# MiroBeno/Volume-Rendering

Hardware: AMD Instinct MI355X
Metric: Mrays/s (W*H / t_frame), 1024^3 volume @ 2048^2 viewport (higher is better)
Workload: dtype f32

## Files before the change

### __graft_entry__.py

```python
import importlib
import os
import subprocess
import sys

ROOT = os.path.dirname(os.path.abspath(__file__))
PKG = "volume-rendering_amd"


def load_package():
    if ROOT not in sys.path:
        sys.path.insert(0, ROOT)
    return importlib.import_module(PKG)


def build():
    subprocess.check_call(["make", "-C", os.path.join(ROOT, PKG, "csrc")])
    os.makedirs(os.path.join(ROOT, "build_variants"), exist_ok=True)
    subprocess.check_call(["bash", os.path.join(ROOT, "scripts", "build_variant.sh"), "bounds", "-DVR_BOUNDS_CHECK"], stdout=subprocess.DEVNULL)
    subprocess.check_call(["make", "-C", os.path.join(ROOT, "oracle"), "oracle"])
    if os.path.isdir("/root/reference/VolumeRendering"):
        subprocess.check_call(["make", "-C", os.path.join(ROOT, "oracle"), "ref"])
        subprocess.check_call(["make", "-C", os.path.join(ROOT, "oracle"), "binding"])
    vr = load_package()
    vr.lib()


def smoke():
    import numpy as np
    import torch

    assert torch.cuda.is_available(), "smoke() needs an MI355X"
    sys.path.insert(0, os.path.join(ROOT, "tests"))
    from helpers import Golden, Oracle, compare_frames
# ... 28 lines not shown
```

### volume-rendering_amd/csrc/vr_device.h

```cpp
#pragma once

#include <hip/hip_runtime.h>
#include <stdint.h>
#include "../../include/vr_hip.h"

namespace vr {

constexpr uint32_t kMaxRaySteps = 1u << 22;

#ifndef VR_DEPTH
#define VR_DEPTH 5
#endif
constexpr int kDepth = VR_DEPTH, kSlots = kDepth + 1;
#ifndef VR_LAZY_EXIT
#define VR_LAZY_EXIT 1
#endif
#ifndef VR_RUN_DEPTH
#define VR_RUN_DEPTH VR_DEPTH
#endif
constexpr int kDepthTwoByte = 3;
constexpr int kRunDepth = VR_RUN_DEPTH, kMaxDepth = kRunDepth > kDepth ? kRunDepth : kDepth;
constexpr int kOverrunSteps = kMaxDepth + (VR_LAZY_EXIT ? kMaxDepth + 1 : 0);
constexpr int kLutPad = (kOverrunSteps * 5 + 2) / 3 + 2;
static_assert(kDepth >= 1 && kDepth <= 6 && kRunDepth >= 1 && kRunDepth <= 12, "prefetch depth");
// ... 140 lines not shown
hipError_t launch_brickify_voxel(const void *linear, void *voxel_bricks, uint32_t bytes_per_voxel, uint32_t dim_x, uint32_t dim_y, uint32_t dim_z,
                                 hipStream_t stream);
hipError_t launch_brickify_oct(const void *linear, void *oct_bricks, uint32_t dim_x, uint32_t dim_y, uint32_t dim_z, hipStream_t stream);
hipError_t launch_brickify_run(const void *linear, void *run_copy, uint32_t run_layout , uint32_t dim_x, uint32_t dim_y,
                               uint32_t dim_z, hipStream_t stream);
hipError_t launch_build_column(const void *linear, void *col_copy, uint32_t axis, bool voxels , uint32_t dim_x, uint32_t dim_y, uint32_t dim_z, hipStream_t stream);
inline uint64_t bricked_elems(uint32_t dim_x, uint32_t dim_y, uint32_t dim_z) {
	return (uint64_t) ((dim_x + kBrickEdge - 1) / kBrickEdge) * ((dim_y + kBrickEdge - 1) / kBrickEdge) *
	       ((dim_z + kBrickEdge - 1) / kBrickEdge) * kBrickPitch;
}

hipError_t launch_raymarch(const RayKernelArgs &a, const void *linear, const void *bricked, uint32_t bytes_per_voxel,
                           const float *tf_premult , const uint32_t *esl_bits ,
                           void *out_rgba, TileSchedule sched, hipStream_t stream);
hipError_t launch_colmarch(const RayKernelArgs &a, const void *copy, const float *tf_premult, void *out_rgba, hipStream_t stream);

struct RaymarchPlan { bool reads_linear; uint32_t tiles_x, tiles_y; uint32_t tile_h = 16;  };
RaymarchPlan plan_raymarch(const RayKernelArgs &a, bool have_bricked, uint32_t bytes_per_voxel);
hipError_t launch_tile_order(uint32_t *cost, uint32_t *order, uint32_t ntiles, hipStream_t stream);
hipError_t launch_tile_estimate(const RayKernelArgs &a, uint32_t tile_h, const uint32_t *esl, uint32_t *cost, uint32_t ntiles, hipStream_t stream);
hipError_t launch_tile_choice(const uint32_t *cost_z, const uint32_t *cost_y, uint32_t *choice, uint32_t ntiles, hipStream_t stream);

hipError_t launch_minmax(const void *volume, uint32_t bytes_per_voxel, uint32_t dim_x, uint32_t dim_y, uint32_t dim_z,
                         uint32_t esl_block_dims, uint8_t *minmax_dev , hipStream_t stream);

constexpr uint32_t kMipBoundEntries = VR_ESL_VOLUME_DIMS * VR_ESL_VOLUME_DIMS * VR_ESL_VOLUME_DIMS;
constexpr uint32_t kMipStatsAt = 2u * kMipBoundEntries + 16u, kMipBoundBytes = kMipStatsAt + 16u;
hipError_t launch_mip_bounds(const uint8_t *minmax_dev , uint8_t *bounds_dev , hipStream_t stream);
hipError_t launch_mip(const RayKernelArgs &a, const void *linear, const void *bricked, uint32_t bytes_per_voxel, const float *tf_premult,
                      const uint8_t *bounds, void *out_rgba, hipStream_t stream);
// ... 12 lines not shown
```

### volume-rendering_amd/csrc/vr_hip_api.cpp

```cpp
#include "vr_device.h"

#include <algorithm>
#include <chrono>
#include <cmath>
#include <cstdio>
#include <cstdlib>
#include <cstring>
#include <new>
#include <string>
#include <vector>

using namespace vr;

#ifndef VR_ORDER_ALWAYS
#define VR_ORDER_ALWAYS 0
#endif

namespace {

constexpr int kEventRing = 256;

struct EventPair { hipEvent_t start = nullptr, stop = nullptr; bool pending = false; };

}
// ... 1249 lines not shown
}

#ifdef VR_MIP_STATS
int vr_hip_debug_mip_stats(vr_ctx *c, uint64_t *out2) {
	if (c == nullptr || out2 == nullptr) return VR_ERR_INVALID;
	out2[0] = out2[1] = 0;
	if (!c->mip_bounds_ready) return VR_OK;
	VR_TRY(c, hipSetDevice(c->device));
	VR_TRY(c, drain(c));
	VR_TRY(c, hipMemcpy(out2, c->mip_bounds + kMipStatsAt, 16, hipMemcpyDeviceToHost));
	VR_TRY(c, hipMemset(c->mip_bounds + kMipStatsAt, 0, 16));
	return VR_OK;
}
#endif

int vr_hip_timing(vr_ctx *c, vr_timing *out) {
	if (c == nullptr || out == nullptr) return VR_ERR_INVALID;
	(void) hipSetDevice(c->device);
	for (int i = 0; i < kEventRing; i++)
		harvest(c, c->ring[(c->ring_head + i) % kEventRing]);
	out->kernel_ms = c->last_kernel_ms;
	out->total_ms = c->last_total_ms > 0 ? c->last_total_ms : c->last_kernel_ms;
	out->launches = c->launches;
	out->kernel_ms_sum = c->kernel_ms_sum;
	out->kernel_ms_max = c->kernel_ms_max;
	out->total_ms_max = c->total_ms_max;
	return VR_OK;
}

int vr_hip_timing_reset(vr_ctx *c) {
// ... 157 lines not shown
```

### volume-rendering_amd/csrc/vr_kernels.hip

```cpp
#include "vr_march.h"

namespace vr {

#ifndef VR_COL_DEPTH
#define VR_COL_DEPTH 3
#endif
#ifndef VR_COL_WAVES
#define VR_COL_WAVES 4
#endif
constexpr int kColDepth = VR_COL_DEPTH, kColSlots = kColDepth + 1;

__device__ __forceinline__ void managed_load128_s(u32x4 &dst, uint32_t byte_offset, uint64_t base) {
	asm volatile("global_load_dwordx4 %0, %1, %2" : "=&v"(dst) : "v"(byte_offset), "s"(base));
}
template <int I> __device__ __forceinline__ float comp3(const f3 &v) { return I == 0 ? v.x : (I == 1 ? v.y : v.z); }

template <int M, bool Q8>
__device__ __forceinline__ float col_resolve(uint32_t w0, uint32_t w1, float max_x, float max_y, float max_z, float xb, float yb, float zb) {
	const float ax = filter_weight<Q8>(__builtin_amdgcn_fractf(__builtin_amdgcn_fmed3f(xb, 0.0f, max_x)));
	const float ay = filter_weight<Q8>(__builtin_amdgcn_fractf(__builtin_amdgcn_fmed3f(yb, 0.0f, max_y)));
	const float az = filter_weight<Q8>(__builtin_amdgcn_fractf(__builtin_amdgcn_fmed3f(zb, 0.0f, max_z)));
	const float p0 = (float) (w0 & 0xffu), p1 = (float) ((w0 >> 8) & 0xffu), p2 = (float) ((w0 >> 16) & 0xffu), p3 = (float) (w0 >> 24);
	const float q0 = (float) (w1 & 0xffu), q1 = (float) ((w1 >> 8) & 0xffu), q2 = (float) ((w1 >> 16) & 0xffu), q3 = (float) (w1 >> 24);
	float v000, v100, v010, v110, v001, v101, v011, v111;
// ... 1 lines not shown
	else if (M == 1) { v000 = p0; v100 = p1; v001 = p2; v101 = p3; v010 = q0; v110 = q1; v011 = q2; v111 = q3; }
	else             { v000 = p0; v010 = p1; v001 = p2; v011 = p3; v100 = q0; v110 = q1; v101 = q2; v111 = q3; }
	const float c00 = lerp(v000, v100, ax), c10 = lerp(v010, v110, ax);
	const float c01 = lerp(v001, v101, ax), c11 = lerp(v011, v111, ax);
	const float c0 = lerp(c00, c10, ay), c1 = lerp(c01, c11, ay);
	return lerp(c0, c1, az);
}


typedef const RayKernelArgs __attribute__((address_space(4))) *ColConstArgs;
struct ColKernelArguments { RayKernelArgs a; const uint8_t *copy; const float *tf_g; uint32_t *out; };
typedef const ColKernelArguments __attribute__((address_space(4))) *ColConstKernelArguments;
__device__ __forceinline__ ColConstArgs col_dense_args() { ColConstArgs q = (ColConstArgs) __builtin_amdgcn_kernarg_segment_ptr(); asm volatile("" : "+s"(q)); return q; }
__device__ __forceinline__ float uni(float v) { return __uint_as_float(rfl(__float_as_uint(v))); }
__device__ __forceinline__ uint32_t col_lane_id() { return __builtin_amdgcn_mbcnt_hi(~0u, __builtin_amdgcn_mbcnt_lo(~0u, 0u)); }

__device__ __forceinline__ void stage_tf_with_deltas(f4 (&tf_l)[VR_TF_SIZE + 1], f4 (&dtf_l)[VR_TF_SIZE + 1], const float *__restrict__ tf_g) {
	const uint32_t t = threadIdx.x;
	if (t <= VR_TF_SIZE) {
		const f4 *tf4 = (const f4 *) tf_g;
		const uint32_t i0 = t < VR_TF_SIZE ? t : VR_TF_SIZE - 1, i1 = t + 1 < VR_TF_SIZE ? t + 1 : VR_TF_SIZE - 1;
		const f4 c0 = tf4[i0], c1 = tf4[i1];
		tf_l[t] = c0;
		f4 d; d.x = c1.x - c0.x; d.y = c1.y - c0.y; d.z = c1.z - c0.z; d.w = c1.w - c0.w;
		dtf_l[t] = d;
	}
}

struct ColRay {
	bool in_frame, alive;
	uint32_t out_index;
	uint32_t org_slot;
	f3 dir, origin;
	float kx, ky, step;
	uint64_t alive_mask;
};
__device__ __forceinline__ f3 col_origin_again(const f4 (&org_l)[512], uint32_t &org_slot) {
	pin(org_slot);
	const f4 o4 = *(const f4 *) ((const char *) org_l + org_slot);
	return mk3(o4.x, o4.y, o4.z);
}
__device__ __forceinline__ void col_ray_setup(const RayKernelArgs &a, f4 (&org_l)[512], ColRay &r) {
	uint32_t tile_x, tile_y;
	tile_to_xy<VR_COL_XCD_MODE>(a.tiles_x, a.tiles_y, blockIdx.x, blockIdx.x, tile_x, tile_y);
	uint32_t lx, ly;
	lane_pixel<512u, true>(a, tile_x, tile_y, lx, ly);
	r.in_frame = lx < a.p.out_width && ly < a.p.out_rows;
	r.out_index = r.in_frame ? ly * a.p.out_width + lx : 0xffffffffu;

	const PixelRay ray = pixel_ray<true>(a, a.p.x0 + lx, frame_row(a, ly));
	r.dir = ray.dir; r.origin = ray.origin;
	r.org_slot = threadIdx.x * (uint32_t) sizeof(f4);
	{ f4 o4; o4.x = r.origin.x; o4.y = r.origin.y; o4.z = r.origin.z; o4.w = 0.0f; org_l[threadIdx.x] = o4; }
	r.kx = ray.kx; r.ky = ray.ky;
	r.step = a.p.ray_step;
	const bool alive = r.in_frame && ray.alive;
	r.alive = alive;
	r.alive_mask = __builtin_amdgcn_ballot_w64(alive);
	if (!alive) r.ky = -1.0f;
}

struct ColWave {
	int leader;
	float kx_l, cm_l;
	int cu0, cv0, cu1, cv1;
	uint64_t flips_u, flips_v;
	bool ok;
};
template <class CellU, class CellV>
__device__ __forceinline__ void col_wave_eligibility(const ColRay &r, float cm, float advance, CellU cell_u, CellV cell_v, ColWave &w) {
	w.leader = __builtin_ctzll(r.alive_mask);
	w.kx_l = rlane(r.kx, w.leader); w.cm_l = rlane(cm, w.leader);
	w.ok = __builtin_amdgcn_ballot_w64(r.alive && (__float_as_uint(r.kx) != __float_as_uint(w.kx_l) || __float_as_uint(cm) != __float_as_uint(w.cm_l))) == 0ull;
	w.ok = w.ok && __builtin_amdgcn_ballot_w64(!(advance >= (1.0f / 64.0f) && advance <= 1.0f)) == 0ull;
	w.cu0 = cell_u(r.kx); w.cv0 = cell_v(r.kx);
	w.cu1 = cell_u(r.ky); w.cv1 = cell_v(r.ky);
	{
		const int lu = __builtin_amdgcn_readlane(w.cu0, w.leader), lv = __builtin_amdgcn_readlane(w.cv0, w.leader);
		if (!r.alive) { w.cu0 = w.cu1 = lu; w.cv0 = w.cv1 = lv; }
	}
	w.flips_u = __builtin_amdgcn_ballot_w64(w.cu0 != w.cu1); w.flips_v = __builtin_amdgcn_ballot_w64(w.cv0 != w.cv1);
	w.ok = w.ok && __builtin_amdgcn_ballot_w64((w.cu1 - w.cu0) * (w.cu1 - w.cu0) > 1 || (w.cv1 - w.cv0) * (w.cv1 - w.cv0) > 1) == 0ull;
}
__device__ __forceinline__ bool col_lane_offsets(const ColWave &w, uint64_t stride_u, uint64_t stride_v, int64_t &ref, int64_t &rel0) {
	ref = (int64_t) col_lateral_offset64((uint32_t) __builtin_amdgcn_readlane(w.cu0, w.leader), (uint32_t) __builtin_amdgcn_readlane(w.cv0, w.leader), stride_u, stride_v);
	rel0 = (int64_t) col_lateral_offset64((uint32_t) w.cu0, (uint32_t) w.cv0, stride_u, stride_v) - ref;
	const int64_t du64 = (int64_t) col_axis_offset64((uint32_t) w.cu1, stride_u, kColWindowBytes) - (int64_t) col_axis_offset64((uint32_t) w.cu0, stride_u, kColWindowBytes);
	const int64_t dv64 = (int64_t) col_axis_offset64((uint32_t) w.cv1, stride_v, kColRowBytes) - (int64_t) col_axis_offset64((uint32_t) w.cv0, stride_v, kColRowBytes);
	const int64_t lim = 1ll << 28;
	return __builtin_amdgcn_ballot_w64(rel0 <= -lim || rel0 >= lim || du64 <= -lim || du64 >= lim || dv64 <= -lim || dv64 >= lim) == 0ull;
}
__device__ __forceinline__ uint64_t col_scalar_base(const uint8_t *copy, int64_t ref) {
	const uint64_t b = (uint64_t) (uintptr_t) copy + (uint64_t) ref - (1ull << 30);
	return ((uint64_t) rfl((uint32_t) (b >> 32)) << 32) | rfl((uint32_t) b);
// ... 198 lines not shown
__device__ __forceinline__ void col_drain(u32x4 (&slot)[N], More &...more) {
	static_for<0, N>([&](auto j) { pin(slot[j.value]); });
	if constexpr (sizeof...(More) != 0) pin(more...);
	managed_wait<0>();
	static_for<0, N>([&](auto j) { pin(slot[j.value]); });
	if constexpr (sizeof...(More) != 0) pin(more...);
}
__device__ __forceinline__ void col_store(const ColRay &ray, const f4 &acc) {
	uint32_t ky_bits = __float_as_uint(ray.ky), out_index = ray.out_index;
	pin(ky_bits, out_index);
	uint32_t rgba = 0;
	if (__uint_as_float(ky_bits) > 0.0f) rgba = map_float_int(acc.x, 256) | (map_float_int(acc.y, 256) << 8) | (map_float_int(acc.z, 256) << 16) | (map_float_int(acc.w, 256) << 24);
	if (out_index != 0xffffffffu) ((ColConstKernelArguments) col_dense_args())->out[out_index] = rgba;
}

template <int SAMPLING, int M, bool FLIPS>
__global__ __launch_bounds__(512) __attribute__((amdgpu_waves_per_eu(VR_COL_WAVES, 8)))
void colmarch_kernel(const RayKernelArgs a, const uint8_t *__restrict__ copy, const float *__restrict__ tf_g, uint32_t *__restrict__ out) {
	constexpr int U = M == 0 ? 1 : 0, V = M == 2 ? 1 : 2;
	__shared__ f4 tf_l[VR_TF_SIZE + 1], dtf_l[VR_TF_SIZE + 1];
	__shared__ f4 org_l[512];
	stage_tf_with_deltas(tf_l, dtf_l, tf_g);
	__syncthreads();
	ColRay ray;
	col_ray_setup(a, org_l, ray);
	if (ray.alive_mask == 0ull) { if (ray.in_frame) out[ray.out_index] = 0u; return; }

	const f3 A = mk3(uni(ray.dir.x * a.half_x), uni(ray.dir.y * a.half_y), uni(ray.dir.z * a.half_z));
	const f3 B = mk3(VR_FMA(ray.origin.x, a.half_x, a.off_x), VR_FMA(ray.origin.y, a.half_y, a.off_y), VR_FMA(ray.origin.z, a.half_z, a.off_z));
	const float Am = comp3<M>(A), Au = comp3<U>(A), Av = comp3<V>(A);
	const float Bm = comp3<M>(B), Bu = comp3<U>(B), Bv = comp3<V>(B);
	const uint32_t dim_u = U == 0 ? a.dim_x : a.dim_y, dim_m = M == 0 ? a.dim_x : (M == 1 ? a.dim_y : a.dim_z);
	const float max_u = U == 0 ? a.max_x : a.max_y, max_v = V == 1 ? a.max_y : a.max_z;
	const uint32_t nbu = col_blocks(dim_u), nw = col_windows(dim_m);
	const uint64_t stride_u = (uint64_t) nw * kColBlockBytes, stride_v = (uint64_t) nbu * stride_u;

	f4 acc; acc.x = acc.y = acc.z = acc.w = 0.0f;
	uint64_t live = ray.alive_mask;
	float k = ray.kx;

	auto coords = [&](ColConstArgs q, float kk, float &xb, float &yb, float &zb) {
// ... 12 lines not shown
		coords(q, kk, xb, yb, zb);
		managed_load64(both, (uint64_t) (uintptr_t) col_pair_address<M>(a, ((ColConstKernelArguments) q)->copy, q->col_sample.max_x, q->col_sample.max_y, q->col_sample.max_z, q->col_shade.nbu, q->col_shade.nw, xb, yb, zb));
	};
	auto sample = [&](uint32_t w0, uint32_t w1) {
		col_tri_sample<SAMPLING, M>(a, w0, w1, k, B, ray, live, acc, tf_l, dtf_l, org_l,
			[&](const uint8_t *copy_p, const RayKernelArgs::ColDenseSample &ds, const RayKernelArgs::ColDenseShade &dh, float sx, float sy, float sz, uint32_t &l0, uint32_t &l1) {
				const uint2 both = *(const uint2 *) col_pair_address<M>(a, copy_p, ds.max_x, ds.max_y, ds.max_z, dh.nbu, dh.nw, sx, sy, sz);
				l0 = both.x; l1 = both.y;
			});
	};

	auto cell = [&](float kk, float Ac, float Bc, float maxc) { return (int) __builtin_amdgcn_fmed3f(VR_FMA(kk, Ac, Bc), 0.0f, maxc); };
	auto cell_u = [&](float kk) { return cell(kk, Au, Bu, max_u); };
	auto cell_v = [&](float kk) { return cell(kk, Av, Bv, max_v); };
	ColWave wv;
	col_wave_eligibility(ray, Bm, __builtin_fabsf(Am) * ray.step, cell_u, cell_v, wv);
	int64_t ref, rel0;
	const bool ok = col_lane_offsets(wv, stride_u, stride_v, ref, rel0) && wv.ok;
	const float Bm_l = wv.cm_l;

	const bool has_flips = (wv.flips_u | wv.flips_v) != 0ull;
	auto per_lane_march = [&]() {
		while (live != 0ull) {
			uint32_t w0, w1;
			fetch_at(k, w0, w1);
			sample(w0, w1);
			k += ray.step;
			live &= __builtin_amdgcn_fcmpf(k, ray.ky, kFcmpOLE);
		}
	};
	if (ok) {
		const uint32_t voff0 = (uint32_t) (rel0 + (1ll << 30));
		const uint64_t s_base = col_scalar_base(copy, ref);
		const int dsign = (__float_as_uint(comp3<M>(ray.dir)) >> 31) != 0u ? -1 : 1;
		auto window_of = [](int lc) { return (int) (__umulhi((uint32_t) lc + 0x30000000u, 0xAAAAAAABu) >> 1) - 0x10000000; };
		auto cell_window = [&](float kk) { return window_of((int) VR_FMA(kk, Am, Bm_l)); };
		int key_u = kColNoEvent, key_v = kColNoEvent;
// ... 39 lines not shown
						} else {
							const uint32_t sub = rfl((uint32_t) (int) VR_FMA(k, Am, Bm_l)) - first;
							sample(sub == 0u ? o.x : (sub == 1u ? o.y : o.z), sub == 0u ? o.y : (sub == 1u ? o.z : o.w));
						}
					});
				}
				cur += dsign;
			};
			while (live != 0ull && guard > 0) {
				static_for<0, kColSlots>(window_step);
				guard -= kColSlots;
			}
			col_drain(slot);
		}
	} else per_lane_march();
	col_store(ray, acc);
}

__device__ __forceinline__ void managed_load8_at(uint32_t &dst, uint64_t address) {
	asm volatile("global_load_ubyte %0, %1, off" : "=&v"(dst) : "v"(address));
}

template <int M, bool FLIPS>
__global__ __launch_bounds__(512) __attribute__((amdgpu_waves_per_eu(VR_COL_WAVES, 8)))
void colmarch_nearest_kernel(const RayKernelArgs a, const uint8_t *__restrict__ copy, const float *__restrict__ tf_g, uint32_t *__restrict__ out) {
	constexpr int U = M == 0 ? 1 : 0, V = M == 2 ? 1 : 2;
	constexpr int kCells = (int) kColVoxCells;
	__shared__ f4 tf_l[VR_TF_SIZE];
	__shared__ float unit_l[256];
	__shared__ f4 org_l[512];
	{
		const uint32_t t = threadIdx.x;
		if (t < VR_TF_SIZE) tf_l[t] = ((const f4 *) tf_g)[t];
		if (t < 256u) unit_l[t] = (float) t / 255.0f;
	}
	__syncthreads();
	ColRay ray;
	col_ray_setup(a, org_l, ray);
	if (ray.alive_mask == 0ull) { if (ray.in_frame) out[ray.out_index] = 0u; return; }

	const float dm = comp3<M>(ray.dir), du = comp3<U>(ray.dir), dv = comp3<V>(ray.dir);
	const float om = comp3<M>(ray.origin), ou = comp3<U>(ray.origin), ov = comp3<V>(ray.origin);
	const uint32_t dim_u = U == 0 ? a.dim_x : a.dim_y, dim_v = V == 1 ? a.dim_y : a.dim_z, dim_m = M == 0 ? a.dim_x : (M == 1 ? a.dim_y : a.dim_z);
	const float half_m = M == 0 ? a.half_x : (M == 1 ? a.half_y : a.half_z);
	const uint32_t nbu = col_blocks(dim_u), nw = col_windows(dim_m, kColVoxCells);
	const uint64_t stride_u = (uint64_t) nw * kColBlockBytes, stride_v = (uint64_t) nbu * stride_u;

	f4 acc; acc.x = acc.y = acc.z = acc.w = 0.0f;
	uint64_t live = ray.alive_mask;
	float k = ray.kx;
	const int opaque_above = ((int) a.tf_zero_below + 1) * VR_TF_RATIO - 1;
	uint32_t near_mask = 0u, near_cmp = 1u;
	if (opaque_above >= 0) { const uint32_t p2 = 1u << (31 - __builtin_clz((uint32_t) opaque_above + 1u)); near_mask = (0xffu & ~(p2 - 1u)) * 0x01010101u; near_cmp = 0u; }

// ... 39 lines not shown
				const float sl = unit_l[s_l], sc = unit_l[s & 255u];
				const float diffuse = select_lanes(shaded, (sl - sc) * kd);
				cur.x += diffuse; cur.y += diffuse; cur.z += diffuse;
			}
			const float t = select_lanes(live, 1 - acc.w);
			acc.x = acc.x + cur.x * t; acc.y = acc.y + cur.y * t;
			acc.z = acc.z + cur.z * t; acc.w = acc.w + cur.w * t;
			live &= ~__builtin_amdgcn_fcmpf(acc.w, threshold, kFcmpOGT);
		}
	};

	auto cell_lat = [&](float kk, float oc, float dc, uint32_t n) { return (int) map_float_int(((oc + dc * kk) + 1) * 0.5f, n); };
	auto cell_u = [&](float kk) { return cell_lat(kk, ou, du, dim_u); };
	auto cell_v = [&](float kk) { return cell_lat(kk, ov, dv, dim_v); };
	ColWave wv;
	col_wave_eligibility(ray, om, __builtin_fabsf(dm * half_m) * ray.step, cell_u, cell_v, wv);
	int64_t ref, rel0;
	const bool ok = col_lane_offsets(wv, stride_u, stride_v, ref, rel0) && wv.ok;
	const float om_l = wv.cm_l;
	auto cell_m = [&](float kk) { const int c = (int) (((om_l + dm * kk) + 1.0f) * half_m); return c == (int) dim_m ? (int) dim_m - 1 : c; };
	const bool has_flips = (wv.flips_u | wv.flips_v) != 0ull;
	auto per_lane_march = [&]() {
		while (live != 0ull) {
			ColConstArgs q = col_dense_args();
			const uint32_t s = *voxel_address_at(q, position(q, k));
			sample(s);
			k += ray.step;
			live &= __builtin_amdgcn_fcmpf(k, ray.ky, kFcmpOLE);
		}
	};
	if (ok) {
		const uint32_t voff0 = (uint32_t) (rel0 + (1ll << 30));
		const uint64_t s_base = col_scalar_base(copy, ref);
		const int dsign = (__float_as_uint(dm) >> 31) != 0u ? -1 : 1;
		auto cell_window = [&](float kk) { return cell_m(kk) >> 4; };
		int key_u = kColNoEvent, key_v = kColNoEvent;
		if (FLIPS && wv.flips_u != 0ull) key_u = wv.cu0 != wv.cu1 ? dsign * cell_window(__uint_as_float(col_bisect(ray, wv.cu0 != wv.cu1, wv.cu0, cell_u))) : kColNoEvent;
// ... 40 lines not shown
							const uint32_t sub = (uint32_t) ((int) rfl((uint32_t) cell_m(k)) - first) & 15u;
							const uint32_t word = (sub >> 2) == 0u ? o.x : ((sub >> 2) == 1u ? o.y : ((sub >> 2) == 2u ? o.z : o.w));
							sample((word >> ((sub & 3u) * 8u)) & 0xffu);
						}
					});
				}
				cur += dsign;
			};
			while (live != 0ull && guard > 0) {
				static_for<0, kColSlots>(window_step);
				guard -= kColSlots;
			}
			col_drain(slot);
		}
	} else per_lane_march();
	col_store(ray, acc);
}

#ifndef VR_VOXCOL_DEPTH
#define VR_VOXCOL_DEPTH 3
#endif
#ifndef VR_VOXCOL_WAVES
#define VR_VOXCOL_WAVES VR_COL_WAVES
#endif
constexpr int kVoxColDepth = VR_VOXCOL_DEPTH, kVoxColSlots = kVoxColDepth + 1;
static_assert(kVoxColDepth >= 2 && 2 * kVoxColSlots + kVoxColDepth + 4 <= 64, "kColPadBytes");

template <int SAMPLING, int M, bool FLIPS, bool PAIRS>
__device__ __forceinline__ void voxcol_march(const RayKernelArgs &a, const uint8_t *__restrict__ copy, const float *__restrict__ tf_g, uint32_t *__restrict__ out,
                                             f4 (&tf_l)[VR_TF_SIZE + 1], f4 (&dtf_l)[VR_TF_SIZE + 1], f4 (&org_l)[512]) {
	constexpr int U = M == 0 ? 1 : 0, V = M == 2 ? 1 : 2;
	constexpr int kCells = (int) kColVoxCells;
	stage_tf_with_deltas(tf_l, dtf_l, tf_g);
	__syncthreads();
	ColRay ray;
	col_ray_setup(a, org_l, ray);
	if (ray.alive_mask == 0ull) { if (ray.in_frame) out[ray.out_index] = 0u; return; }

	const f3 A = mk3(uni(ray.dir.x * a.half_x), uni(ray.dir.y * a.half_y), uni(ray.dir.z * a.half_z));
	const f3 B = mk3(VR_FMA(ray.origin.x, a.half_x, a.off_x), VR_FMA(ray.origin.y, a.half_y, a.off_y), VR_FMA(ray.origin.z, a.half_z, a.off_z));
	const float Am = comp3<M>(A), Au = comp3<U>(A), Av = comp3<V>(A);
	const float Bm = comp3<M>(B), Bu = comp3<U>(B), Bv = comp3<V>(B);
	const uint32_t dim_u = U == 0 ? a.dim_x : a.dim_y, dim_v = V == 1 ? a.dim_y : a.dim_z, dim_m = M == 0 ? a.dim_x : (M == 1 ? a.dim_y : a.dim_z);
	const float max_u = U == 0 ? a.max_x : a.max_y, max_v = V == 1 ? a.max_y : a.max_z;
	const uint32_t nbu = col_blocks(dim_u), nw = col_windows(dim_m, kColVoxCells);
	const uint64_t stride_u = (uint64_t) nw * kColBlockBytes, stride_v = (uint64_t) nbu * stride_u;

	f4 acc; acc.x = acc.y = acc.z = acc.w = 0.0f;
	uint64_t live = ray.alive_mask;
	float k = ray.kx;

	auto corners_at = [&](const uint8_t *copy_p, float mx, float my, float mz, uint32_t blocks_u, uint32_t windows, float xb, float yb, float zb,
	                      uint32_t &w0, uint32_t &w1) {
		if constexpr (PAIRS) {
			const uint2 both = *(const uint2 *) col_pair_address<M>(a, copy_p, mx, my, mz, blocks_u, windows, xb, yb, zb);
			w0 = both.x; w1 = both.y;
			return;
		}
		const uint32_t ix = (uint32_t) (int) __builtin_amdgcn_fmed3f(xb, 0.0f, mx), iy = (uint32_t) (int) __builtin_amdgcn_fmed3f(yb, 0.0f, my),
		               iz = (uint32_t) (int) __builtin_amdgcn_fmed3f(zb, 0.0f, mz);
		const float fu = U == 0 ? mx : my, fv = V == 1 ? my : mz, fm = M == 0 ? mx : (M == 1 ? my : mz);
		const uint32_t iu = U == 0 ? ix : iy, iv = V == 1 ? iy : iz, im = M == 0 ? ix : (M == 1 ? iy : iz);
		const uint32_t iu1 = iu + ((float) iu < fu ? 1u : 0u), iv1 = iv + ((float) iv < fv ? 1u : 0u), im1 = im + ((float) im < fm ? 1u : 0u);
		auto along = [](uint32_t m) { return (m >> 4) * kColBlockBytes + (m & 15u); };
// ... 4 lines not shown
		w1 = ld(l00 + m1) | (ld(l10 + m1) << 8) | (ld(l01 + m1) << 16) | (ld(l11 + m1) << 24);
	};
	auto fetch_at = [&](float kk, uint32_t &w0, uint32_t &w1) {
		ColConstArgs q = col_dense_args();
		const float xb = VR_FMA(kk, q->col_sample.ax, B.x), yb = VR_FMA(kk, q->col_sample.ay, B.y), zb = VR_FMA(kk, q->col_sample.az, B.z);
		corners_at(PAIRS ? (const uint8_t *) (uintptr_t) q->alt_copy : ((ColConstKernelArguments) q)->copy, q->col_sample.max_x, q->col_sample.max_y, q->col_sample.max_z,
		           q->col_shade.nbu, PAIRS ? q->col_shade.nwq : q->col_shade.nw, xb, yb, zb, w0, w1);
	};
	auto sample = [&](uint32_t w0, uint32_t w1) {
		col_tri_sample<SAMPLING, M, PAIRS>(a, w0, w1, k, B, ray, live, acc, tf_l, dtf_l, org_l,
			[&](const uint8_t *copy_p, const RayKernelArgs::ColDenseSample &ds, const RayKernelArgs::ColDenseShade &dh, float sx, float sy, float sz, uint32_t &l0, uint32_t &l1) {
				corners_at(copy_p, ds.max_x, ds.max_y, ds.max_z, dh.nbu, dh.nw, sx, sy, sz, l0, l1);
			});
	};

	auto cell = [&](float kk, float Ac, float Bc, float maxc) { return (int) __builtin_amdgcn_fmed3f(VR_FMA(kk, Ac, Bc), 0.0f, maxc); };
	auto cell_u = [&](float kk) { return cell(kk, Au, Bu, max_u); };
	auto cell_v = [&](float kk) { return cell(kk, Av, Bv, max_v); };
	ColWave wv;
	col_wave_eligibility(ray, Bm, __builtin_fabsf(Am) * ray.step, cell_u, cell_v, wv);
	const float Bm_l = wv.cm_l;
	const int cu0 = wv.cu0, cu1 = wv.cu1, cv0 = wv.cv0, cv1 = wv.cv1;
	const uint64_t flips = wv.flips_u | wv.flips_v;
	bool ok = wv.ok && (FLIPS || flips == 0ull);
	int ru0 = cu0 < cu1 ? cu0 : cu1, ru1 = (cu0 > cu1 ? cu0 : cu1) + 1, rv0 = cv0 < cv1 ? cv0 : cv1, rv1 = (cv0 > cv1 ? cv0 : cv1) + 1;
	#pragma unroll
	for (int d = 32; d >= 1; d >>= 1) {
		const int a0 = __shfl_xor(ru0, d, 64), a1 = __shfl_xor(ru1, d, 64), a2 = __shfl_xor(rv0, d, 64), a3 = __shfl_xor(rv1, d, 64);
		ru0 = a0 < ru0 ? a0 : ru0; ru1 = a1 > ru1 ? a1 : ru1; rv0 = a2 < rv0 ? a2 : rv0; rv1 = a3 > rv1 ? a3 : rv1;
	}
	ru0 = (int) rfl((uint32_t) ru0); ru1 = (int) rfl((uint32_t) ru1); rv0 = (int) rfl((uint32_t) rv0); rv1 = (int) rfl((uint32_t) rv1);
	const int rw = ru1 - ru0 + 1, nrect = rw * (rv1 - rv0 + 1);
	ok = ok && nrect <= 64;
	const uint32_t lane_i = col_lane_id();
	int own_u, own_v;
	{
		const int j = (int) lane_i < nrect ? (int) lane_i : nrect - 1;
		const int jv = j / rw;
		own_u = ru0 + (j - jv * rw); own_v = rv0 + jv;
		own_u = own_u < (int) dim_u - 1 ? own_u : (int) dim_u - 1; own_v = own_v < (int) dim_v - 1 ? own_v : (int) dim_v - 1;
	}
	const int64_t ref = (int64_t) col_lateral_offset64((uint32_t) ru0, (uint32_t) rv0, stride_u, stride_v);
	const int64_t rel = (int64_t) col_lateral_offset64((uint32_t) own_u, (uint32_t) own_v, stride_u, stride_v) - ref;
	ok = ok && __builtin_amdgcn_ballot_w64(rel < 0 || rel >= (1ll << 28)) == 0ull;

	auto per_lane_march = [&]() {
		while (live != 0ull) {
			uint32_t w0, w1;
			fetch_at(k, w0, w1);
			sample(w0, w1);
			k += ray.step;
			live &= __builtin_amdgcn_fcmpf(k, ray.ky, kFcmpOLE);
		}
	};
	if (ok) {
		const uint32_t voff = (uint32_t) (rel + (1ll << 30));
		const uint64_t s_base = col_scalar_base(copy, ref);
		const int dsign = (__float_as_uint(comp3<M>(ray.dir)) >> 31) != 0u ? -1 : 1;
		const bool forward = dsign > 0;
		const uint32_t rw4 = (uint32_t) rw * 4u;
		const uint32_t own0 = (uint32_t) ((cu0 - ru0) + (cv0 - rv0) * rw) * 4u;
		float t_u = __builtin_inff(), t_v = __builtin_inff();
		uint32_t step_u = 0u, step_v = 0u;
		if (FLIPS && flips != 0ull) {
			const uint32_t bu = col_bisect(ray, cu0 != cu1, cu0, cell_u), bv = col_bisect(ray, cv0 != cv1, cv0, cell_v);
			t_u = cu0 != cu1 ? __uint_as_float(bu) : __builtin_inff();
			t_v = cv0 != cv1 ? __uint_as_float(bv) : __builtin_inff();
			step_u = (uint32_t) (cu1 - cu0) * 4u; step_v = (uint32_t) (cv1 - cv0) * rw4;
		}
		auto cell_window = [&](float kk) { return (int) VR_FMA(kk, Am, Bm_l) >> 4; };
		ColBatch batch = { 0.0f, wv.kx_l, 0 };
		auto next_batch = [&]() { batch.refill(ray.step, lane_i, cell_window); };
		next_batch();
// ... 41 lines not shown
					const uint32_t p00 = (uint32_t) __builtin_amdgcn_ds_bpermute((int) at, pair), p10 = (uint32_t) __builtin_amdgcn_ds_bpermute((int) (at + 4u), pair);
					const uint32_t p01 = (uint32_t) __builtin_amdgcn_ds_bpermute((int) (at + rw4), pair), p11 = (uint32_t) __builtin_amdgcn_ds_bpermute((int) (at + rw4 + 4u), pair);
					const uint32_t t0 = __builtin_amdgcn_perm(p10, p00, 0x05010400u), t1 = __builtin_amdgcn_perm(p11, p01, 0x05010400u);
					sample(__builtin_amdgcn_perm(t1, t0, 0x05040100u), __builtin_amdgcn_perm(t1, t0, 0x07060302u));
				});
			}
			carry = o.x;
			cur += dsign;
		};
		while (live != 0ull && guard > 0) {
			static_for<0, kVoxColSlots>(window_step);
			guard -= kVoxColSlots;
		}
		col_drain(slot, carry);
	} else per_lane_march();
	col_store(ray, acc);
}

template <int SAMPLING, int M, bool FLIPS>
__global__ __launch_bounds__(512) __attribute__((amdgpu_waves_per_eu(VR_VOXCOL_WAVES, 8)))
void voxcol_tri_kernel(const RayKernelArgs a, const uint8_t *__restrict__ copy, const float *__restrict__ tf_g, uint32_t *__restrict__ out) {
	__shared__ f4 tf_l[VR_TF_SIZE + 1], dtf_l[VR_TF_SIZE + 1];
	__shared__ f4 org_l[512];
	voxcol_march<SAMPLING, M, FLIPS, false>(a, copy, tf_g, out, tf_l, dtf_l, org_l);
}
template <int SAMPLING, int M, bool FLIPS>
__global__ __launch_bounds__(512) __attribute__((amdgpu_waves_per_eu(VR_VOXCOL_WAVES, 8)))
void voxcol_pairs_kernel(const RayKernelArgs a, const uint8_t *__restrict__ copy, const float *__restrict__ tf_g, uint32_t *__restrict__ out) {
	__shared__ f4 tf_l[VR_TF_SIZE + 1], dtf_l[VR_TF_SIZE + 1];
	__shared__ f4 org_l[512];
// ... 26 lines not shown
```

Before: 2239.

## Split voxcol waves into up to four coherent ray groups and add column stats

```diff
diff --git a/__graft_entry__.py b/__graft_entry__.py
--- a/__graft_entry__.py
+++ b/__graft_entry__.py
@@ -17,6 +17,7 @@
     subprocess.check_call(["make", "-C", os.path.join(ROOT, PKG, "csrc")])
     os.makedirs(os.path.join(ROOT, "build_variants"), exist_ok=True)
     subprocess.check_call(["bash", os.path.join(ROOT, "scripts", "build_variant.sh"), "bounds", "-DVR_BOUNDS_CHECK"], stdout=subprocess.DEVNULL)
+    subprocess.check_call(["bash", os.path.join(ROOT, "scripts", "build_variant.sh"), "colstats", "-DVR_COL_STATS"], stdout=subprocess.DEVNULL)
     subprocess.check_call(["make", "-C", os.path.join(ROOT, "oracle"), "oracle"])
     if os.path.isdir("/root/reference/VolumeRendering"):
         subprocess.check_call(["make", "-C", os.path.join(ROOT, "oracle"), "ref"])
diff --git a/volume-rendering_amd/csrc/vr_device.h b/volume-rendering_amd/csrc/vr_device.h
--- a/volume-rendering_amd/csrc/vr_device.h
+++ b/volume-rendering_amd/csrc/vr_device.h
@@ -178,6 +178,11 @@
                            const float *tf_premult , const uint32_t *esl_bits ,
                            void *out_rgba, TileSchedule sched, hipStream_t stream);
 hipError_t launch_colmarch(const RayKernelArgs &a, const void *copy, const float *tf_premult, void *out_rgba, hipStream_t stream);
+#ifdef VR_COL_STATS
+struct ColStatRecord { uint32_t cls, passes; uint64_t cycles, wall_start, wall_end; };
+constexpr uint32_t kColStatRecords = 131072u;
+hipError_t col_stats_fetch(uint64_t *counts4, ColStatRecord *records, uint32_t max_records);
+#endif
 
 struct RaymarchPlan { bool reads_linear; uint32_t tiles_x, tiles_y; uint32_t tile_h = 16;  };
 RaymarchPlan plan_raymarch(const RayKernelArgs &a, bool have_bricked, uint32_t bytes_per_voxel);
diff --git a/volume-rendering_amd/csrc/vr_hip_api.cpp b/volume-rendering_amd/csrc/vr_hip_api.cpp
--- a/volume-rendering_amd/csrc/vr_hip_api.cpp
+++ b/volume-rendering_amd/csrc/vr_hip_api.cpp
@@ -1287,6 +1287,16 @@
 }
 #endif
 
+#ifdef VR_COL_STATS
+int vr_hip_debug_col_stats(vr_ctx *c, uint64_t *counts4, void *records, uint32_t max_records) {
+	if (c == nullptr || counts4 == nullptr) return VR_ERR_INVALID;
+	VR_TRY(c, hipSetDevice(c->device));
+	VR_TRY(c, drain(c));
+	VR_TRY(c, col_stats_fetch(counts4, (ColStatRecord *) records, max_records));
+	return VR_OK;
+}
+#endif
+
 int vr_hip_timing(vr_ctx *c, vr_timing *out) {
 	if (c == nullptr || out == nullptr) return VR_ERR_INVALID;
 	(void) hipSetDevice(c->device);
diff --git a/volume-rendering_amd/csrc/vr_kernels.hip b/volume-rendering_amd/csrc/vr_kernels.hip
--- a/volume-rendering_amd/csrc/vr_kernels.hip
+++ b/volume-rendering_amd/csrc/vr_kernels.hip
@@ -39,6 +39,8 @@
 __device__ __forceinline__ ColConstArgs col_dense_args() { ColConstArgs q = (ColConstArgs) __builtin_amdgcn_kernarg_segment_ptr(); asm volatile("" : "+s"(q)); return q; }
 __device__ __forceinline__ float uni(float v) { return __uint_as_float(rfl(__float_as_uint(v))); }
 __device__ __forceinline__ uint32_t col_lane_id() { return __builtin_amdgcn_mbcnt_hi(~0u, __builtin_amdgcn_mbcnt_lo(~0u, 0u)); }
+__device__ __forceinline__ uint32_t col_pass_lane_id() { uint32_t lane = col_lane_id(); asm volatile("" : "+v"(lane)); return lane; }
+__device__ __forceinline__ int col_shfl_xor(int v, uint32_t lane, int d) { return __builtin_amdgcn_ds_bpermute((int) ((lane ^ (uint32_t) d) << 2), v); }
 
 __device__ __forceinline__ void stage_tf_with_deltas(f4 (&tf_l)[VR_TF_SIZE + 1], f4 (&dtf_l)[VR_TF_SIZE + 1], const float *__restrict__ tf_g) {
 	const uint32_t t = threadIdx.x;
@@ -65,6 +67,10 @@
 	const f4 o4 = *(const f4 *) ((const char *) org_l + org_slot);
 	return mk3(o4.x, o4.y, o4.z);
 }
+__device__ __forceinline__ float col_kx_again(const f4 (&org_l)[512], uint32_t &org_slot) {
+	pin(org_slot);
+	return *(const float *) ((const char *) org_l + org_slot + 12u);
+}
 __device__ __forceinline__ void col_ray_setup(const RayKernelArgs &a, f4 (&org_l)[512], ColRay &r) {
 	uint32_t tile_x, tile_y;
 	tile_to_xy<VR_COL_XCD_MODE>(a.tiles_x, a.tiles_y, blockIdx.x, blockIdx.x, tile_x, tile_y);
@@ -76,7 +82,7 @@
 	const PixelRay ray = pixel_ray<true>(a, a.p.x0 + lx, frame_row(a, ly));
 	r.dir = ray.dir; r.origin = ray.origin;
 	r.org_slot = threadIdx.x * (uint32_t) sizeof(f4);
-	{ f4 o4; o4.x = r.origin.x; o4.y = r.origin.y; o4.z = r.origin.z; o4.w = 0.0f; org_l[threadIdx.x] = o4; }
+	{ f4 o4; o4.x = r.origin.x; o4.y = r.origin.y; o4.z = r.origin.z; o4.w = ray.kx; org_l[threadIdx.x] = o4; }
 	r.kx = ray.kx; r.ky = ray.ky;
 	r.step = a.p.ray_step;
 	const bool alive = r.in_frame && ray.alive;
@@ -85,24 +91,34 @@
 	if (!alive) r.ky = -1.0f;
 }
 
+constexpr int kColMaxGroups = 4;
 struct ColWave {
 	int leader;
 	float kx_l, cm_l;
 	int cu0, cv0, cu1, cv1;
+	uint64_t group;
 	uint64_t flips_u, flips_v;
 	bool ok;
 };
-template <class CellU, class CellV>
-__device__ __forceinline__ void col_wave_eligibility(const ColRay &r, float cm, float advance, CellU cell_u, CellV cell_v, ColWave &w) {
-	w.leader = __builtin_ctzll(r.alive_mask);
+template <int MAX_GROUPS, class CellU, class CellV>
+__device__ __forceinline__ void col_wave_eligibility(const ColRay &r, uint64_t todo, float cm, float advance, CellU cell_u, CellV cell_v, ColWave &w) {
+	auto same_as = [&](int lane) {
+		return __builtin_amdgcn_ballot_w64(__float_as_uint(r.kx) == __float_as_uint(rlane(r.kx, lane)) && __float_as_uint(cm) == __float_as_uint(rlane(cm, lane)));
+	};
+	w.leader = __builtin_ctzll(todo);
 	w.kx_l = rlane(r.kx, w.leader); w.cm_l = rlane(cm, w.leader);
-	w.ok = __builtin_amdgcn_ballot_w64(r.alive && (__float_as_uint(r.kx) != __float_as_uint(w.kx_l) || __float_as_uint(cm) != __float_as_uint(w.cm_l))) == 0ull;
+	w.group = same_as(w.leader) & todo;
+	uint64_t rest = todo & ~w.group;
+	for (int g = 1; g < MAX_GROUPS && rest != 0ull; g++) rest &= ~same_as(__builtin_ctzll(rest));
+	w.ok = rest == 0ull;
+	if (!w.ok) w.group = todo;
+	const bool member = ((w.group >> col_lane_id()) & 1ull) != 0ull;
 	w.ok = w.ok && __builtin_amdgcn_ballot_w64(!(advance >= (1.0f / 64.0f) && advance <= 1.0f)) == 0ull;
 	w.cu0 = cell_u(r.kx); w.cv0 = cell_v(r.kx);
 	w.cu1 = cell_u(r.ky); w.cv1 = cell_v(r.ky);
 	{
 		const int lu = __builtin_amdgcn_readlane(w.cu0, w.leader), lv = __builtin_amdgcn_readlane(w.cv0, w.leader);
-		if (!r.alive) { w.cu0 = w.cu1 = lu; w.cv0 = w.cv1 = lv; }
+		if (!member) { w.cu0 = w.cu1 = lu; w.cv0 = w.cv1 = lv; }
 	}
 	w.flips_u = __builtin_amdgcn_ballot_w64(w.cu0 != w.cu1); w.flips_v = __builtin_amdgcn_ballot_w64(w.cv0 != w.cv1);
 	w.ok = w.ok && __builtin_amdgcn_ballot_w64((w.cu1 - w.cu0) * (w.cu1 - w.cu0) > 1 || (w.cv1 - w.cv0) * (w.cv1 - w.cv0) > 1) == 0ull;
@@ -331,6 +347,45 @@
 	if (out_index != 0xffffffffu) ((ColConstKernelArguments) col_dense_args())->out[out_index] = rgba;
 }
 
+#ifdef VR_COL_STATS
+__device__ unsigned long long g_col_stat_counts[4];
+__device__ ColStatRecord g_col_stat_records[kColStatRecords];
+struct ColStats {
+	__device__ __forceinline__ ColStatRecord *record() const {
+		const uint32_t wave = blockIdx.x * 8u + threadIdx.x / 64u;
+		return col_lane_id() == 0u && wave < kColStatRecords ? &g_col_stat_records[wave] : nullptr;
+	}
+	__device__ __forceinline__ void begin() const {
+		if (ColStatRecord *r = record()) { r->cls = 0u; r->passes = 0u; r->cycles = __builtin_readcyclecounter(); r->wall_start = wall_clock64(); }
+		managed_wait<0>();
+	}
+	__device__ __forceinline__ void pass() const { if (ColStatRecord *r = record()) r->passes = r->passes + 1u; managed_wait<0>(); }
+	__device__ __forceinline__ void per_lane() const { if (ColStatRecord *r = record()) r->cls = 1u; managed_wait<0>(); }
+	__device__ __forceinline__ void end() const {
+		if (ColStatRecord *r = record()) {
+			const uint32_t cls = r->cls != 0u ? 1u : (r->passes > 1u ? 2u : 0u);
+			r->cls = cls; r->cycles = __builtin_readcyclecounter() - r->cycles; r->wall_end = wall_clock64();
+			atomicAdd(&g_col_stat_counts[cls], 1ull);
+			atomicAdd(&g_col_stat_counts[3], 1ull);
+		}
+	}
+};
+hipError_t col_stats_fetch(uint64_t *counts4, ColStatRecord *records, uint32_t max_records) {
+	hipError_t e = hipMemcpyFromSymbol(counts4, HIP_SYMBOL(g_col_stat_counts), 4 * sizeof(uint64_t));
+	const uint32_t n = max_records < kColStatRecords ? max_records : kColStatRecords;
+	if (e == hipSuccess && records != nullptr && n != 0u) e = hipMemcpyFromSymbol(records, HIP_SYMBOL(g_col_stat_records), (size_t) n * sizeof(ColStatRecord));
+	void *p = nullptr;
+	if (e == hipSuccess) e = hipGetSymbolAddress(&p, HIP_SYMBOL(g_col_stat_counts));
+	if (e == hipSuccess) e = hipMemset(p, 0, 4 * sizeof(uint64_t));
+	if (e == hipSuccess) e = hipGetSymbolAddress(&p, HIP_SYMBOL(g_col_stat_records));
+	if (e == hipSuccess) e = hipMemset(p, 0, sizeof(ColStatRecord) * kColStatRecords);
+	return e;
+}
+#define VR_COL_STAT(...) __VA_ARGS__
+#else
+#define VR_COL_STAT(...)
+#endif
+
 template <int SAMPLING, int M, bool FLIPS>
 __global__ __launch_bounds__(512) __attribute__((amdgpu_waves_per_eu(VR_COL_WAVES, 8)))
 void colmarch_kernel(const RayKernelArgs a, const uint8_t *__restrict__ copy, const float *__restrict__ tf_g, uint32_t *__restrict__ out) {
@@ -342,6 +397,7 @@
 	ColRay ray;
 	col_ray_setup(a, org_l, ray);
 	if (ray.alive_mask == 0ull) { if (ray.in_frame) out[ray.out_index] = 0u; return; }
+	VR_COL_STAT(ColStats stats; stats.begin(); stats.pass();)
 
 	const f3 A = mk3(uni(ray.dir.x * a.half_x), uni(ray.dir.y * a.half_y), uni(ray.dir.z * a.half_z));
 	const f3 B = mk3(VR_FMA(ray.origin.x, a.half_x, a.off_x), VR_FMA(ray.origin.y, a.half_y, a.off_y), VR_FMA(ray.origin.z, a.half_z, a.off_z));
@@ -384,13 +440,14 @@
 	auto cell_u = [&](float kk) { return cell(kk, Au, Bu, max_u); };
 	auto cell_v = [&](float kk) { return cell(kk, Av, Bv, max_v); };
 	ColWave wv;
-	col_wave_eligibility(ray, Bm, __builtin_fabsf(Am) * ray.step, cell_u, cell_v, wv);
+	col_wave_eligibility<1>(ray, ray.alive_mask, Bm, __builtin_fabsf(Am) * ray.step, cell_u, cell_v, wv);
 	int64_t ref, rel0;
 	const bool ok = col_lane_offsets(wv, stride_u, stride_v, ref, rel0) && wv.ok;
 	const float Bm_l = wv.cm_l;
 
 	const bool has_flips = (wv.flips_u | wv.flips_v) != 0ull;
 	auto per_lane_march = [&]() {
+		VR_COL_STAT(stats.per_lane();)
 		while (live != 0ull) {
 			uint32_t w0, w1;
 			fetch_at(k, w0, w1);
@@ -460,6 +517,7 @@
 			col_drain(slot);
 		}
 	} else per_lane_march();
+	VR_COL_STAT(stats.end();)
 	col_store(ray, acc);
 }
 
@@ -484,6 +542,7 @@
 	ColRay ray;
 	col_ray_setup(a, org_l, ray);
 	if (ray.alive_mask == 0ull) { if (ray.in_frame) out[ray.out_index] = 0u; return; }
+	VR_COL_STAT(ColStats stats; stats.begin(); stats.pass();)
 
 	const float dm = comp3<M>(ray.dir), du = comp3<U>(ray.dir), dv = comp3<V>(ray.dir);
 	const float om = comp3<M>(ray.origin), ou = comp3<U>(ray.origin), ov = comp3<V>(ray.origin);
@@ -553,13 +612,14 @@
 	auto cell_u = [&](float kk) { return cell_lat(kk, ou, du, dim_u); };
 	auto cell_v = [&](float kk) { return cell_lat(kk, ov, dv, dim_v); };
 	ColWave wv;
-	col_wave_eligibility(ray, om, __builtin_fabsf(dm * half_m) * ray.step, cell_u, cell_v, wv);
+	col_wave_eligibility<1>(ray, ray.alive_mask, om, __builtin_fabsf(dm * half_m) * ray.step, cell_u, cell_v, wv);
 	int64_t ref, rel0;
 	const bool ok = col_lane_offsets(wv, stride_u, stride_v, ref, rel0) && wv.ok;
 	const float om_l = wv.cm_l;
 	auto cell_m = [&](float kk) { const int c = (int) (((om_l + dm * kk) + 1.0f) * half_m); return c == (int) dim_m ? (int) dim_m - 1 : c; };
 	const bool has_flips = (wv.flips_u | wv.flips_v) != 0ull;
 	auto per_lane_march = [&]() {
+		VR_COL_STAT(stats.per_lane();)
 		while (live != 0ull) {
 			ColConstArgs q = col_dense_args();
 			const uint32_t s = *voxel_address_at(q, position(q, k));
@@ -630,6 +690,7 @@
 			col_drain(slot);
 		}
 	} else per_lane_march();
+	VR_COL_STAT(stats.end();)
 	col_store(ray, acc);
 }
 
@@ -647,23 +708,19 @@
                                              f4 (&tf_l)[VR_TF_SIZE + 1], f4 (&dtf_l)[VR_TF_SIZE + 1], f4 (&org_l)[512]) {
 	constexpr int U = M == 0 ? 1 : 0, V = M == 2 ? 1 : 2;
 	constexpr int kCells = (int) kColVoxCells;
+	constexpr bool GROUPS = PAIRS;
 	stage_tf_with_deltas(tf_l, dtf_l, tf_g);
 	__syncthreads();
 	ColRay ray;
 	col_ray_setup(a, org_l, ray);
 	if (ray.alive_mask == 0ull) { if (ray.in_frame) out[ray.out_index] = 0u; return; }
-
-	const f3 A = mk3(uni(ray.dir.x * a.half_x), uni(ray.dir.y * a.half_y), uni(ray.dir.z * a.half_z));
+	VR_COL_STAT(ColStats stats; stats.begin();)
+
 	const f3 B = mk3(VR_FMA(ray.origin.x, a.half_x, a.off_x), VR_FMA(ray.origin.y, a.half_y, a.off_y), VR_FMA(ray.origin.z, a.half_z, a.off_z));
-	const float Am = comp3<M>(A), Au = comp3<U>(A), Av = comp3<V>(A);
 	const float Bm = comp3<M>(B), Bu = comp3<U>(B), Bv = comp3<V>(B);
-	const uint32_t dim_u = U == 0 ? a.dim_x : a.dim_y, dim_v = V == 1 ? a.dim_y : a.dim_z, dim_m = M == 0 ? a.dim_x : (M == 1 ? a.dim_y : a.dim_z);
-	const float max_u = U == 0 ? a.max_x : a.max_y, max_v = V == 1 ? a.max_y : a.max_z;
-	const uint32_t nbu = col_blocks(dim_u), nw = col_windows(dim_m, kColVoxCells);
-	const uint64_t stride_u = (uint64_t) nw * kColBlockBytes, stride_v = (uint64_t) nbu * stride_u;
 
 	f4 acc; acc.x = acc.y = acc.z = acc.w = 0.0f;
-	uint64_t live = ray.alive_mask;
+	uint64_t live = 0ull;
 	float k = ray.kx;
 
 	auto corners_at = [&](const uint8_t *copy_p, float mx, float my, float mz, uint32_t blocks_u, uint32_t windows, float xb, float yb, float zb,
@@ -698,19 +755,46 @@
 			});
 	};
 
+	auto per_lane_march = [&]() {
+		VR_COL_STAT(stats.per_lane();)
+		while (live != 0ull) {
+			uint32_t w0, w1;
+			fetch_at(k, w0, w1);
+			sample(w0, w1);
+			k += ray.step;
+			live &= __builtin_amdgcn_fcmpf(k, ray.ky, kFcmpOLE);
+		}
+	};
+
+	uint64_t todo = ray.alive_mask;
+	do {
+	ColConstArgs qa = col_dense_args();
+	const f3 A = mk3(uni(qa->p.view.direction[0] * qa->half_x), uni(qa->p.view.direction[1] * qa->half_y), uni(qa->p.view.direction[2] * qa->half_z));
+	const float Am = comp3<M>(A), Au = comp3<U>(A), Av = comp3<V>(A);
+	const uint32_t dim_u = U == 0 ? qa->dim_x : qa->dim_y, dim_v = V == 1 ? qa->dim_y : qa->dim_z, dim_m = M == 0 ? qa->dim_x : (M == 1 ? qa->dim_y : qa->dim_z);
+	const float max_u = U == 0 ? qa->max_x : qa->max_y, max_v = V == 1 ? qa->max_y : qa->max_z;
+	const uint32_t nbu = col_blocks(dim_u), nw = col_windows(dim_m, kColVoxCells);
+	const uint64_t stride_u = (uint64_t) nw * kColBlockBytes, stride_v = (uint64_t) nbu * stride_u;
+	VR_COL_STAT(stats.pass();)
+	ray.kx = col_kx_again(org_l, ray.org_slot);
+
 	auto cell = [&](float kk, float Ac, float Bc, float maxc) { return (int) __builtin_amdgcn_fmed3f(VR_FMA(kk, Ac, Bc), 0.0f, maxc); };
 	auto cell_u = [&](float kk) { return cell(kk, Au, Bu, max_u); };
 	auto cell_v = [&](float kk) { return cell(kk, Av, Bv, max_v); };
 	ColWave wv;
-	col_wave_eligibility(ray, Bm, __builtin_fabsf(Am) * ray.step, cell_u, cell_v, wv);
+	col_wave_eligibility<GROUPS ? kColMaxGroups : 1>(ray, todo, Bm, __builtin_fabsf(Am) * ray.step, cell_u, cell_v, wv);
+	live = wv.group;
+	todo &= ~wv.group;
+	k = ray.kx;
 	const float Bm_l = wv.cm_l;
 	const int cu0 = wv.cu0, cu1 = wv.cu1, cv0 = wv.cv0, cv1 = wv.cv1;
 	const uint64_t flips = wv.flips_u | wv.flips_v;
 	bool ok = wv.ok && (FLIPS || flips == 0ull);
 	int ru0 = cu0 < cu1 ? cu0 : cu1, ru1 = (cu0 > cu1 ? cu0 : cu1) + 1, rv0 = cv0 < cv1 ? cv0 : cv1, rv1 = (cv0 > cv1 ? cv0 : cv1) + 1;
+	const uint32_t lane_p = col_pass_lane_id();
 	#pragma unroll
 	for (int d = 32; d >= 1; d >>= 1) {
-		const int a0 = __shfl_xor(ru0, d, 64), a1 = __shfl_xor(ru1, d, 64), a2 = __shfl_xor(rv0, d, 64), a3 = __shfl_xor(rv1, d, 64);
+		const int a0 = col_shfl_xor(ru0, lane_p, d), a1 = col_shfl_xor(ru1, lane_p, d), a2 = col_shfl_xor(rv0, lane_p, d), a3 = col_shfl_xor(rv1, lane_p, d);
 		ru0 = a0 < ru0 ? a0 : ru0; ru1 = a1 > ru1 ? a1 : ru1; rv0 = a2 < rv0 ? a2 : rv0; rv1 = a3 > rv1 ? a3 : rv1;
 	}
 	ru0 = (int) rfl((uint32_t) ru0); ru1 = (int) rfl((uint32_t) ru1); rv0 = (int) rfl((uint32_t) rv0); rv1 = (int) rfl((uint32_t) rv1);
@@ -728,19 +812,10 @@
 	const int64_t rel = (int64_t) col_lateral_offset64((uint32_t) own_u, (uint32_t) own_v, stride_u, stride_v) - ref;
 	ok = ok && __builtin_amdgcn_ballot_w64(rel < 0 || rel >= (1ll << 28)) == 0ull;
 
-	auto per_lane_march = [&]() {
-		while (live != 0ull) {
-			uint32_t w0, w1;
-			fetch_at(k, w0, w1);
-			sample(w0, w1);
-			k += ray.step;
-			live &= __builtin_amdgcn_fcmpf(k, ray.ky, kFcmpOLE);
-		}
-	};
 	if (ok) {
 		const uint32_t voff = (uint32_t) (rel + (1ll << 30));
-		const uint64_t s_base = col_scalar_base(copy, ref);
-		const int dsign = (__float_as_uint(comp3<M>(ray.dir)) >> 31) != 0u ? -1 : 1;
+		const uint64_t s_base = col_scalar_base(((ColConstKernelArguments) qa)->copy, ref);
+		const int dsign = (__float_as_uint(qa->p.view.direction[M]) >> 31) != 0u ? -1 : 1;
 		const bool forward = dsign > 0;
 		const uint32_t rw4 = (uint32_t) rw * 4u;
 		const uint32_t own0 = (uint32_t) ((cu0 - ru0) + (cv0 - rv0) * rw) * 4u;
@@ -812,6 +887,8 @@
 		}
 		col_drain(slot, carry);
 	} else per_lane_march();
+	} while (GROUPS && todo != 0ull);
+	VR_COL_STAT(stats.end();)
 	col_store(ray, acc);
 }
 
```

Result: no change. 2250, median of 6 (+0.5%).
